# mozendr/FHE-SPEAR

Hardware: AMD Instinct MI355X
Metric: BSGS matvecs/sec at d=2048,N=16384,L0=36; sec/RWKV-block at 1/2/4/8 GPU (higher is better)
Workload: dtype u64

## Files before the change

fhe-spear_amd/csrc/fhs_host.hip:

```cpp
#include <execinfo.h>
#include <hip/hip_runtime.h>
#include <unistd.h>

#include <algorithm>
#include <csignal>
#include <atomic>
#include <cmath>
#include <complex>
#include <cstdio>
#include <cstring>
#include <map>
#include <unordered_map>
#include <chrono>
#include <memory>
#include <mutex>
#include <set>
#include <string>
#include <thread>
#include <vector>

#include "../../include/fhespear.h"
#include "fhs_kernels.h"
#include "fhs_modarith.h"
#include "fhs_tables.h"
// ... 47 lines not shown
    if (!bits || !out || n <= 0 || N < 2 || (N & (N - 1))) return fail(FHS_ERR_INVALID, "create_coeff_modulus: bad args");
    for (int i = 0; i < n; ++i)
        if (bits[i] < 2 || bits[i] > 61) return fail(FHS_ERR_INVALID, "create_coeff_modulus: bit size must be in [2, 61]");
    if (!coeff_modulus_search(N, bits, n, out)) return fail(FHS_ERR_INVALID, "create_coeff_modulus: not enough primes");
    return FHS_OK;
}
extern "C" uint64_t fhs_galois_elt_from_step(int step, uint64_t N) { return galois_elt_from_step(step, N); }

struct PendingRot {
    KsItem item;
    fhs_ciphertext* out;
    const fhs_ciphertext* in;
};

struct fhs_context {
    int device = 0;
    hipStream_t st = nullptr;
    fhs::KsSide side{};
    std::recursive_mutex mu;
    uint64_t N = 0;
    int logN = 0, L0 = 0, P = 0, K = 0, dnum = 0;
    std::vector<uint64_t> q;
    std::vector<uint64_t> elts;
    DevTables T{};
    std::vector<void*> tables;
    void* items_dev = nullptr;
    void* ptrs_dev = nullptr;
    std::vector<PendingRot> pending;
    int pending_l = -1;
    std::set<const void*> pending_refs;
    std::set<const void*> pending_outs;
    int debug_fail_flushes = 0;
    int debug_fail_alloc = -1;
    std::vector<std::complex<double>> fft_w;
    std::vector<std::complex<double>> dec_twist;
    std::vector<uint64_t> slot_index;
    std::atomic<uint64_t> bytes_live{0};
    std::atomic<int> refs{1};
    std::unordered_map<size_t, std::vector<void*>> free_blocks;
    std::unordered_map<const void*, uint64_t*> key_a;
    size_t cached_bytes = 0;
    size_t cache_cap = 0;
    uint64_t cache_tick = 0;
    std::unordered_map<size_t, uint64_t> size_tick;
    uint64_t evicted_blocks = 0, fit_hits = 0, seal_corr_drops = 0;
    uint32_t timer_mask = 0;
    std::vector<hipEvent_t> timer_open;
    std::vector<std::vector<std::pair<hipEvent_t, hipEvent_t>>> timer_pairs;
    fhs::KTimer ktimer{};
    unsigned char* ring = nullptr;
    size_t ring_head = 0;
    int ring_seg = 0;
    static constexpr size_t kRingBytes = 16u << 20;
    static constexpr int kRingSegs = 8;
    static constexpr size_t kSegBytes = kRingBytes / kRingSegs;
    hipEvent_t ring_ev[kRingSegs] = {};
    uint64_t ring_waits = 0, ring_blocked = 0;
    fhs::Stager stager{};
    std::map<std::pair<int, int>, std::vector<uint64_t>> crt_cache;
    double* readback = nullptr;
    size_t readback_bytes = 0;
    std::map<std::pair<const uint64_t*, int>, uint64_t*> seal_corr;
    size_t seal_corr_bytes = 0;
    size_t seal_corr_cap = 0;
    fhs::SealHoist seal_hoist{};
    enum { SCR_KS, SCR_BSGS_INNER, SCR_BSGS_WS, SCR_BSGS_SUM, SCR_RESCALE, SCR_ENC_PTRS, SCR_COUNT };
// ... 1185 lines not shown
    return export_dev(c, pd, pt_bytes(pt), host);
}
extern "C" fhs_status fhs_ciphertext_import(fhs_context* c, const uint64_t* host, int ncomp, int ci, double scale,
                                            fhs_ciphertext** out) {
    ENTER(c);
    if (!host || !out || ncomp < 2 || ncomp > 3) return fail(FHS_ERR_INVALID, "ciphertext_import: bad args");
    NEW_CT(ct, ncomp, ci, scale);
    HIPCHK(hipMemcpyAsync(ct->d, host, ct_bytes(ct.p), hipMemcpyHostToDevice, c->st), "ciphertext_import");
    HIPCHK(hipStreamSynchronize(c->st), "ciphertext_import");
    *out = ct.release();
    return FHS_OK;
}
extern "C" fhs_status fhs_plaintext_import(fhs_context* c, const uint64_t* host, int ci, double scale,
                                           fhs_plaintext** out) {
    ENTER(c);
    if (!host || !out) return fail(FHS_ERR_INVALID, "plaintext_import: bad args");
    NEW_PT(pt, ci, scale);
    HIPCHK(hipMemcpyAsync(pt->d, host, pt_bytes(pt.p), hipMemcpyHostToDevice, c->st), "plaintext_import");
    HIPCHK(hipStreamSynchronize(c->st), "plaintext_import");
    *out = pt.release();
    return FHS_OK;
}
extern "C" fhs_status fhs_debug_fail_next_flushes(fhs_context* c, int count) {
    if (!c || count < 0) return fail(FHS_ERR_INVALID, "debug_fail_next_flushes: bad args");
    Guard g(c);
    c->debug_fail_flushes = count;
    return FHS_OK;
}
extern "C" fhs_status fhs_debug_force_fork(fhs_context* c, int on, uint64_t* forked) {
    if (!c) return fail(FHS_ERR_INVALID, "debug_force_fork: null context");
    Guard g(c);
    if (on >= 0) c->side.min_wg = on ? 0 : fhs::kForkMinWg;
    if (forked) *forked = c->side.forked;
    return FHS_OK;
}
extern "C" fhs_status fhs_debug_fail_alloc(fhs_context* c, int nth, int* was_armed) {
    if (!c) return fail(FHS_ERR_INVALID, "debug_fail_alloc: null context");
    Guard g(c);
    if (was_armed) *was_armed = c->debug_fail_alloc >= 0;
    c->debug_fail_alloc = nth < 0 ? -1 : nth;
    return FHS_OK;
}
extern "C" fhs_status fhs_debug_alloc_stats(fhs_context* c, uint64_t* out, int n) {
    if (!c || !out || n < 0) return fail(FHS_ERR_INVALID, "debug_alloc_stats: bad args");
    Guard g(c);
    const uint64_t v[FHS_ALLOC_STATS_COUNT] = {c->cached_bytes,    c->cache_cap,     c->evicted_blocks, c->fit_hits,
                                               c->seal_corr_bytes, c->seal_corr_cap, c->seal_corr_drops};
    for (int i = 0; i < n && i < FHS_ALLOC_STATS_COUNT; ++i) out[i] = v[i];
    return FHS_OK;
}
extern "C" fhs_status fhs_debug_launch_ledger(int op, char* buf, uint64_t len, uint64_t* needed) {
    if (op == FHS_LEDGER_ARM || op == FHS_LEDGER_DISARM) {
        fhs::ledger_arm(op == FHS_LEDGER_ARM);
        return FHS_OK;
    }
    if (op != FHS_LEDGER_READ) return fail(FHS_ERR_INVALID, "debug_launch_ledger: unknown operation");
    const std::string names = fhs::ledger_read();
    if (needed) *needed = names.size() + 1;
    if (!buf || len < names.size() + 1) return fail(FHS_ERR_INVALID, "debug_launch_ledger: buffer too short");
    memcpy(buf, names.c_str(), names.size() + 1);
    return FHS_OK;
}
extern "C" fhs_status fhs_ciphertext_device_ptr(const fhs_ciphertext* ct, void** dptr, uint64_t* bytes) {
    if (!ct || !dptr) return fail(FHS_ERR_INVALID, "null argument");
    fhs_context* c = ct->ctx;
    Guard g(c);
// ... 1204 lines not shown
        if (!baby[b] || baby[b]->l != l || baby[b]->ncomp != 2 || baby[b]->ci != ci)
            return fail(FHS_ERR_LEVEL, "bsgs: baby steps and diagonals must share one chain index");
        LIVE(baby[b]);
    }
    if (rescale && l < 2) return fail(FHS_ERR_LEVEL, "bsgs: no level left for the final rescale");
    if (giant_elts && giant_elts[0] != 1) return fail(FHS_ERR_INVALID, "linear_transform: giant group 0 must be the identity");
    HostTrace ht;
    std::vector<const uint64_t*> keys(Beff, nullptr), akeys(Beff, nullptr);
    for (int g = 1; g < Beff; ++g) {
        const uint64_t elt = giant_elts ? giant_elts[g] : fhs_galois_elt_from_step(g * G, c->N);
        auto it = gk->keys.find(elt);
        if (it == gk->keys.end()) return fail(FHS_ERR_KEY, "bsgs: galois key for a giant step is missing");
        keys[g] = it->second;
        akeys[g] = key_akey(c, it->second);
    }
    const size_t S = (size_t)l * c->N;
    std::vector<const uint64_t*> ptrs(G + D);
    for (int b = 0; b < G; ++b) ptrs[b] = baby[b]->d;
    for (int k = 0; k < D; ++k) ptrs[G + k] = pt_ptrs[k];
    ht.mark("keys+ptrs");
    HIPCHK(stage_h2d(c, c->ptrs_dev, ptrs.data(), sizeof(void*) * (G + D)), "bsgs");
    ht.mark("stage ptrs");
    const uint64_t* const* dbaby = reinterpret_cast<const uint64_t* const*>(c->ptrs_dev);
    const uint64_t* const* dpts = dbaby + G;
    uint64_t* inner = nullptr;
    HIPCHK(scratch(c, fhs_context::SCR_BSGS_INNER, 8ull * Beff * 2 * S, &inner), "bsgs inner products");
    const fhs::KTimer* tm = ktimer(c);
    const size_t wsb = std::max<size_t>(8, fhs::bsgs_workspace_bytes(c->T, Beff - 1, l));
    uint64_t* ws = nullptr;
    HIPCHK(scratch(c, fhs_context::SCR_BSGS_WS, wsb, &ws), "bsgs workspace");
    uint64_t* sum = nullptr;
    HIPCHK(scratch(c, fhs_context::SCR_BSGS_SUM, 16 * S, &sum), "bsgs sum");
    ht.mark("workspaces");
    HIPCHK(fhs::launch_bsgs(c->T, dbaby, dpts, G, Beff, D, l, keys.data(), akeys.data(), giant_elts, inner, sum, ws, wsb,
                            c->items_dev, c->stager, c->st, tm, ptl, &c->side),
           "bsgs");
    ht.mark("launch bsgs");
    if (!rescale) {
        NEW_CT(r, 2, ci, baby[0]->scale * pt_scale);
        HIPCHK(hipMemcpyAsync(r->d, sum, 8 * 2 * S, hipMemcpyDeviceToDevice, c->st), "linear_transform");
        *out = r.release();
        return FHS_OK;
    }
    NEW_CT(r, 2, ci + 1, baby[0]->scale * pt_scale / (double)c->q[l - 1]);
    uint64_t* scr = nullptr;
    HIPCHK(scratch(c, fhs_context::SCR_RESCALE, 16ull * c->N, &scr), "bsgs rescale");
    HIPCHK(fhs::launch_rescale(c->T, sum, r->d, scr, 2, l, c->st, tm), "bsgs rescale");
    ht.mark("rescale+frees");
    *out = r.release();
    return FHS_OK;
}

static int pts_ptl(const fhs_context* c, const fhs_plaintext* const* pts, int D) {
    static const bool dense = getenv("FHESPEAR_BSGS_DENSE") != nullptr;
    if (dense || D < 1 || c->T.max_qbits > 59 || !pts[0]->dc) return 0;
    for (int k = 1; k < D; ++k)
        if (!pts[k]->dc || pts[k]->tlog != pts[0]->tlog) return 0;
    return pts[0]->tlog;
}
extern "C" fhs_status fhs_bsgs_multiply_accumulate(fhs_context* c, const fhs_ciphertext* const* baby, int G,
                                                   const fhs_plaintext* const* pts, int D, int B,
                                                   const fhs_galois_keys* gk, fhs_ciphertext** out) {
    ENTER(c);
    if (!pts || !gk || !out || !baby) return fail(FHS_ERR_INVALID, "null argument");
    std::vector<const uint64_t*> p(D);
    for (int k = 0; k < D; ++k) {
// ... 893 lines not shown
```

fhe-spear_amd/csrc/fhs_kernels.h:

```cpp
#pragma once
#include <hip/hip_runtime.h>
#include <stdint.h>

#include <string>

struct PrfKey;

namespace fhs {

typedef uint64_t u64;

struct DevTables {
    const void* primes;
    const u64* tw_fwd;
    const u64* tw_inv;
    const u64* modup_intt;
    const u64* modup_hat;
    const u64* modup_R;
    const u64* modup_Q;
    const u64* modup_xd;
    const u64* modup_xt;
    const u64* md_xd;
    const u64* md_intt;
    const u64* md_hat;
// ... 54 lines not shown

hipError_t launch_ntt_fwd(const DevTables& T, u64* data, int limbs, int l_split, int npoly, size_t poly_stride,
                          hipStream_t st);
hipError_t launch_ntt_inv(const DevTables& T, u64* data, int limbs, int l_split, int npoly, size_t poly_stride,
                          hipStream_t st);
hipError_t launch_eltwise(const DevTables& T, int op, const u64* a, const u64* b, u64* out, int ncomp, int l,
                          size_t a_cstride, size_t b_cstride, hipStream_t st);
hipError_t launch_tensor(const DevTables& T, const u64* const* a_dev, const u64* const* b_dev, const u64* a, const u64* b,
                         int R, u64* out3, int l, hipStream_t st);
hipError_t launch_rescale(const DevTables& T, const u64* in, u64* out, u64* scratch, int ncomp, int l,
                          hipStream_t st, const KTimer* tm = nullptr);
hipError_t launch_rescale_many(const DevTables& T, const u64* const* ins_dev, const u64* const* mul_dev, int count, int l,
                               u64* out, u64* scratch, hipStream_t st, const KTimer* tm = nullptr);
struct Stager {
    void* user;
    hipError_t (*h2d)(void* user, void* dst, const void* src, size_t bytes);
};
constexpr int kForkMinWg = 8 * 256;
struct KsSide {
    hipStream_t st = nullptr;
    hipEvent_t fork = nullptr, join = nullptr;
    int min_wg = kForkMinWg;
    unsigned long long forked = 0;
};
hipError_t launch_keyswitch(const DevTables& T, const KsItem* items_host, int R, const u64* const* uniq_host, int U,
                            int l, u64* workspace, size_t ws_bytes, void* items_dev, const Stager& sg, hipStream_t st,
                            const KTimer* tm, SealHoist* sh = nullptr);
size_t keyswitch_workspace_bytes(const DevTables& T, int R, int U, int l);

size_t bsgs_workspace_bytes(const DevTables& T, int R, int l);
hipError_t launch_bsgs(const DevTables& T, const u64* const* baby_dev, const u64* const* pts_dev, int G, int B, int D,
                       int l, const u64* const* keys_host, const u64* const* akeys_host, const u64* giant_elts, u64* inner,
                       u64* out, u64* workspace, size_t ws_bytes, void* items_dev, const Stager& sg, hipStream_t st,
                       const KTimer* tm, int ptl = 0, KsSide* side = nullptr);
hipError_t launch_bsgs_inner(const DevTables& T, const u64* const* baby_dev, const u64* const* pts_dev, int G, int g0,
                             int g1, int D, int l, u64* inner, hipStream_t st, int ptl = 0);
hipError_t launch_dot_tensor(const DevTables& T, const u64* const* q_dev, const u64* const* db_dev, int J, int C, int l,
                             u64* out3, hipStream_t st, const KTimer* tm = nullptr);
hipError_t launch_encode(const DevTables& T, const double* vals, int count, size_t n, size_t stride, bool is_real,
                         double scale, u64* const* outs_dev, int l, hipStream_t st,
                         double* coef_scratch = nullptr, const unsigned char* tlog = nullptr,
                         u64* const* couts_dev = nullptr, int ss = 0);
hipError_t launch_enc_period(const double* vals, int count, size_t n, size_t stride, bool is_real, int smax,
                             unsigned char* tlog, hipStream_t st);
int encode_sparse_max_log(int logN);
hipError_t launch_expand_compact(const u64* dc, u64* d, int l, int N, int tl, hipStream_t st);
hipError_t launch_sample(const DevTables& T, int mode, const ::PrfKey& K, u64 sid, u64* out, int l, hipStream_t st,
                         int npoly = 1, u64 sid_step = 0, u64* const* outs_dev = nullptr);
hipError_t launch_switch_key_assemble(const DevTables& T, u64* b_out, const u64* a, const u64* e_ntt, const u64* s_ntt,
                                      const u64* snew_ntt, int digit, hipStream_t st);
hipError_t launch_galois_perm(const DevTables& T, const u64* in, u64* out, int limbs, u64 elt, hipStream_t st);
hipError_t launch_encrypt_sym_batch(const DevTables& T, const ::PrfKey& K, u64 sid_mask, u64 sid_err, u64 sid_step,
                                    u64* const* cts_dev, const u64* s, const u64* const* pts_dev, int count, int l,
                                    signed char* small, u64* eb, hipStream_t st, const double* coef = nullptr);
hipError_t launch_encode_coef(const DevTables& T, const double* vals, int count, size_t n, size_t stride, bool is_real,
                              double scale, double* coef, hipStream_t st, const unsigned char* tlog = nullptr);
hipError_t launch_encrypt_pk_batch(const DevTables& T, const ::PrfKey& K, u64 sid, u64 sid_step, u64* cts,
                                   const u64* pk0, const u64* pk1, const u64* const* pts_dev, const u64* pt,
                                   const double* coef, int count, int l, signed char* small, u64* ub, hipStream_t st,
                                   const KTimer* tm = nullptr);
hipError_t launch_encrypt_combine(const DevTables& T, int mode, u64* c0, u64* c1, const u64* s_or_pk0, const u64* pk1,
                                  const u64* u_ntt, const u64* e0, const u64* e1, const u64* pt, int l, hipStream_t st);
hipError_t launch_decrypt(const DevTables& T, const u64* ct, int ncomp, const u64* s, u64* out, int l, hipStream_t st);
hipError_t launch_decrypt_many(const DevTables& T, const u64* const* cts_dev, int count, int ncomp, const u64* s, u64* out,
                               size_t out_stride, int l, hipStream_t st);
hipError_t launch_diag_gather(const double* M1, const double* M2, int D, int G, int n, int k0, int rows, int trans,
                              double* out, hipStream_t st);
// ... 54 lines not shown
```

fhe-spear_amd/csrc/fhs_kernels.hip:

```cpp
#include "fhs_kernels.h"
typedef unsigned long long u64x2_t __attribute__((ext_vector_type(2)));
#ifndef FHS_MODUP_STORE_AUX
#define FHS_MODUP_STORE_AUX 2
#endif
#ifndef FHS_KSIP_UNROLL
#define FHS_KSIP_UNROLL 4
#endif
#include "fhs_ntt.h"
#include "fhs_buffer.h"
#include "fhs_xcdmap.h"

#include <atomic>
#include <cxxabi.h>
#include <mutex>
#include <set>
#include <string>
#include <cstdio>
#include <cstdlib>
#include <cstring>
#include <vector>
#include <algorithm>

#define FHS_INNER_WAVES 16
#define FHS_INNER_VEC 2
// ... 471 lines not shown
    const int vecs = wg2 >= 8 * 256 ? 2 : 1;
    FHS_LAUNCH(k_tensor, dim3((T.N + 512 * vecs - 1) / (512 * vecs), l, R), dim3(256), 0, st, T, a_dev, b_dev, a, b, out3, l,
               vecs);
    return hipGetLastError();
}

__global__ void k_key_prod(DevTables T, const u64* a, const u64* b, u64* out, int limbs) {
    const size_t S = (size_t)limbs * T.N;
    for (size_t idx = blockIdx.x * (size_t)blockDim.x + threadIdx.x; idx < S; idx += (size_t)gridDim.x * blockDim.x) {
        const PrimeK& P = PK(T, (int)(idx / T.N));
        out[idx] = mulmod(a[idx], b[idx], P);
    }
}
hipError_t launch_key_prod(const DevTables& T, const u64* a, const u64* b, u64* out, int limbs, hipStream_t st) {
    FHS_LAUNCH(k_key_prod, dim3(eltwise_grid((size_t)limbs * T.N)), dim3(256), 0, st, T, a, b, out, limbs);
    return hipGetLastError();
}

__global__ void k_galois_perm(DevTables T, const u64* in, u64* out, int limbs, u64 elt) {
    const size_t S = (size_t)limbs * T.N;
    for (size_t idx = blockIdx.x * (size_t)blockDim.x + threadIdx.x; idx < S; idx += (size_t)gridDim.x * blockDim.x) {
        const size_t base = idx - idx % T.N;
        out[idx] = in[base + galois_src((int)(idx % T.N), elt, T.logN)];
    }
}
hipError_t launch_galois_perm(const DevTables& T, const u64* in, u64* out, int limbs, u64 elt, hipStream_t st) {
    FHS_LAUNCH(k_galois_perm, dim3(eltwise_grid((size_t)limbs * T.N)), dim3(256), 0, st, T, in, out, limbs,
               elt);
    return hipGetLastError();
}

template <int LOGN, bool H = ntt_half<LOGN>()>
__global__ void __launch_bounds__((ntt_threads<LOGN, H>())) k_rescale_intt(DevTables T, const u64* in, const u64* const* ins,
                                                                      const u64* const* mul, u64* scratch, int l) {
    constexpr int N = 1 << LOGN;
    __shared__ __attribute__((aligned(16))) u64 lds[ntt_lds_words<LOGN, H>()];
    const int comp = blockIdx.x, pi = l - 1;
    const PrimeK& P = PK(T, pi);
    const u64* src = ins ? ins[comp >> 1] + ((size_t)(comp & 1) * l + pi) * N : in + ((size_t)comp * l + pi) * N;
    u64* dst = scratch + (size_t)comp * N;
    const u64 half = P.q >> 1, q = P.q;
    const u64* tw = T.tw_inv + (size_t)pi * N * 2;
    auto store = [&](int e, u64 v) { dst[e] = addmod(v, half, q); };
    if (mul) {
        const u64* pt = mul[comp >> 1] + (size_t)pi * N;
        inv_limb<LOGN, FHS_NTT_RL, H>(lds, threadIdx.x, tw, q, P.ninv, P.ninv_s, P.w1ninv, P.w1ninv_s,
                                   [&](int e) { return mulmod(src[e], pt[e], P); }, store);
    } else {
        inv_limb<LOGN, FHS_NTT_RL, H>(lds, threadIdx.x, tw, q, P.ninv, P.ninv_s, P.w1ninv, P.w1ninv_s,
                                   [&](int e) { return src[e]; }, store);
    }
}
template <int LOGN, bool H = ntt_half<LOGN>()>
__global__ void __launch_bounds__((ntt_threads<LOGN, H>())) k_rescale_ntt(DevTables T, const u64* in, const u64* const* ins,
                                                                     const u64* const* mul, const u64* scratch, u64* out,
                                                                     int l) {
    constexpr int N = 1 << LOGN;
    __shared__ __attribute__((aligned(16))) u64 lds[ntt_lds_words<LOGN, H>()];
    const int i = blockIdx.x, comp = blockIdx.y;
    const PrimeK& P = PK(T, i);
    const RedU RU = redu(P);
    const u64* rs = T.rescale + ((size_t)l * T.L0 + i) * 4;
    const u64 inv = rs[0], inv_s = rs[1], hq = rs[2], q = RU.q;
    const u64* src = scratch + (size_t)comp * N;
    const u64* a = ins ? ins[comp >> 1] + ((size_t)(comp & 1) * l + i) * N : in + ((size_t)comp * l + i) * N;
    u64* o = out + ((size_t)comp * (l - 1) + i) * N;
    const u64* tw = T.tw_fwd + (size_t)i * N * 2;
    auto load = [&](int e) { return submod(reduce64(src[e], P), hq, q); };
    if (mul) {
        const u64* pt = mul[comp >> 1] + (size_t)i * N;
        fwd_limb<LOGN, FHS_NTT_RL, H>(lds, threadIdx.x, tw, RU, load, [&](int e, u64 t) {
            o[e] = shoup(submod(mulmod(a[e], pt[e], P), t, q), inv, inv_s, q);
        });
    } else {
        fwd_limb<LOGN, FHS_NTT_RL, H>(lds, threadIdx.x, tw, RU, load,
                                   [&](int e, u64 t) { o[e] = shoup(submod(a[e], t, q), inv, inv_s, q); });
    }
// ... 60 lines not shown
    if constexpr (WLX) {
        const int wb = wl_base<LOGN - 1, 16, 8>(tid), wp = lds_pad(wb);
#pragma unroll
        for (int c = 0; c < 16; ++c) {
            const int off = wl_off<LOGN - 1, 16, 8>(c);
            const int e = g * NH + wb + off;
            o[e] = shoup(submod(a[e], fwd_canon(lds[wp + off + off / 16], RU), q), inv, inv_s, q);
        }
    } else {
#pragma unroll
        for (int c = 0; c < 16; ++c) {
            const int e = g * NH + tid + c * TH;
            o[e] = shoup(submod(a[e], fwd_canon(lds[row_pad<TH>(tid, c)], RU), q), inv, inv_s, q);
        }
    }
}
#ifndef FHS_SPLIT_MAX_WG
#define FHS_SPLIT_MAX_WG 256
#endif
hipError_t launch_rescale(const DevTables& T, const u64* in, u64* out, u64* scratch, int ncomp, int l,
                          hipStream_t st, const KTimer* tm) {
    FHS_TMARK(tm, KID_RESCALE, 1, st);
    FHS_DISPATCH_LOGN(T.logN, {
        if constexpr (LOGN == 15) {
            if (ncomp <= 2) {
                FHS_LAUNCH((k_rescale_intt_hs<LOGN>), dim3(2, ncomp), dim3(ntt_threads<LOGN, true>()), 0, st, T,
                           in, scratch, l);
                FHS_LAUNCH((k_rescale_ntt_hs<LOGN>), dim3(l - 1, ncomp, 2), dim3(ntt_threads<LOGN, true>()), 0, st,
                           T, in, scratch, out, l);
                break;
            }
        }
        constexpr const u64* const* none = nullptr;
        FHS_NTT_LAUNCH(k_rescale_intt, ncomp, dim3(ncomp), st, T, in, none, none, scratch, l);
        FHS_NTT_LAUNCH(k_rescale_ntt, (l - 1) * ncomp, dim3(l - 1, ncomp), st, T, in, none, none, scratch, out, l);
    });
    FHS_TMARK(tm, KID_RESCALE, 0, st);
    return hipGetLastError();
}

hipError_t launch_rescale_many(const DevTables& T, const u64* const* ins_dev, const u64* const* mul_dev, int count, int l,
                               u64* out, u64* scratch, hipStream_t st, const KTimer* tm) {
    if (!ins_dev || count < 1 || 2 * (size_t)count > 65535 || l < 2 || l > 65536) return hipErrorInvalidValue;
    const int ncomp = 2 * count;
    FHS_TMARK(tm, KID_RESCALE, 1, st);
    FHS_DISPATCH_LOGN(T.logN, {
        constexpr const u64* none = nullptr;
        FHS_NTT_LAUNCH(k_rescale_intt, ncomp, dim3(ncomp), st, T, none, ins_dev, mul_dev, scratch, l);
        FHS_NTT_LAUNCH(k_rescale_ntt, (l - 1) * ncomp, dim3(l - 1, ncomp), st, T, none, ins_dev, mul_dev, scratch, out, l);
    });
    FHS_TMARK(tm, KID_RESCALE, 0, st);
    return hipGetLastError();
}

hipError_t launch_last_limbs_intt(const DevTables& T, const u64* const* ins_dev, int count, int l, u64* dco, hipStream_t st,
                                  const KTimer* tm) {
    if (count < 1 || count > 65535 || l < 1) return hipErrorInvalidValue;
    FHS_TMARK(tm, KID_WSUM_INTT, 1, st);
    FHS_DISPATCH_LOGN(T.logN, {
        FHS_NTT_LAUNCH(k_rescale_intt, 2 * count, dim3(2 * count), st, T, static_cast<const u64*>(nullptr), ins_dev,
                       static_cast<const u64* const*>(nullptr), dco, l);
    });
    FHS_TMARK(tm, KID_WSUM_INTT, 0, st);
    return hipGetLastError();
}

template <int LOGN>
__global__ void __launch_bounds__((1 << LOGN) / 16) k_ks_intt(DevTables T, const u64* const* uniq, u64* acoef, int l, int U) {
    constexpr int N = 1 << LOGN, TH = N / 16;
    __shared__ __attribute__((aligned(16))) u64 lds[ntt_lds_words<LOGN, false>()];
    const int tid = threadIdx.x;
    int i, u;
    if (!plain_tm(blockIdx.x, l, U, i, u)) return;
    const PrimeK& P = PK(T, i);
    const u64* src = uniq[u] + (size_t)i * N;
#pragma unroll
    for (int c = 0; c < 16; ++c) lds[row_pad<TH>(tid, c)] = src[tid + c * TH];
    __syncthreads();
    const u64* cst = T.modup_intt + ((size_t)l * T.L0 + i) * 4;
    ntt_inv_lds<LOGN, FHS_NTT_RL>(lds, tid, T.tw_inv + (size_t)i * N * 2, P.q, cst[0], cst[1], cst[2], cst[3]);
    u64* dst = acoef + ((size_t)u * l + i) * N;
#pragma unroll
    for (int k = 0; k < 16; ++k) dst[tid + k * TH] = csub(lds[row_pad<TH>(tid, k)], P.q);
}

template <int LOGN>
__global__ void __launch_bounds__((1 << LOGN) / 32, 4) k_ks_intt_h(DevTables T, const u64* const* uniq, u64* acoef,
                                                                   int l, int U) {
    constexpr int N = 1 << LOGN, NH = N / 2, TH = N / 32;
    __shared__ __attribute__((aligned(16))) u64 lds[(1 << (LOGN - 1)) + (1 << (LOGN - 1)) / 16];
    const int tid = threadIdx.x;
    int i, u;
    if (!plain_tm(blockIdx.x, l, U, i, u)) return;
    const PrimeK& P = PK(T, i);
// ... 1253 lines not shown
        }
#pragma unroll
        for (int j = 0; j < FHS_GSUM_RB; ++j) {
#pragma unroll
            for (int k = 0; k < PMAX; ++k) {
                if (k < P_) {
                    ylo[k] += v[j][k];
                    yhi[k] += ylo[k] < v[j][k];
                }
            }
        }
    }
    for (int i = i0; i < i1; ++i) {
        const PrimeK& P = PK(T, i);
        const u64 q = P.q;
        u128 cs = {0, 0};
#pragma unroll
        for (int k = 0; k < PMAX; ++k)
            if (k < P_) mac128(cs, reduce128(ylo[k], yhi[k], P), T.md_hat[(size_t)k * T.L0 + i]);
        if (T.ks_seal) {
            u128 h = {0, 0};
            mac128(h, (u64)R, T.md_pinv[3 * T.L0 + i]);
            const u64 rh = reduce128(h.lo, h.hi, P);
            cs.lo = reduce128(cs.lo, cs.hi, P);
            cs.hi = 0;
            cs.lo = submod(cs.lo, rh, q);
        }
        u64 cv = reduce128(cs.lo, cs.hi, P);
        convsum[(size_t)comp * S + (size_t)i * N + n] = cv;
    }
}
template <int LOGN, bool H = ntt_half<LOGN>()>
__global__ void __launch_bounds__((ntt_threads<LOGN, H>())) k_giant_final(DevTables T, const u64* bpart, const u64* inner0,
                                                                     const u64* convsum, u64* out, int l) {
    constexpr int N = 1 << LOGN;
    __shared__ __attribute__((aligned(16))) u64 lds[ntt_lds_words<LOGN, H>()];
    const int i = blockIdx.x, comp = blockIdx.y;
    const PrimeK& P = PK(T, i);
    const RedU RU = redu(P);
    const size_t off = ((size_t)comp * l + i) * N, boff = ((size_t)comp * (l + T.P) + i) * N;
    const u64 pinv = T.md_pinv[2 * i], pinv_s = T.md_pinv[2 * i + 1], q = RU.q;
    fwd_limb<LOGN, FHS_NTT_RL, H>(lds, threadIdx.x, T.tw_fwd + (size_t)i * N * 2, RU,
                               [&](int e) { return convsum[off + e]; },
                               [&](int e, u64 v) {
                                   out[off + e] = submod(addmod(bpart[boff + e], inner0[off + e], q),
                                                         shoup(v, pinv, pinv_s, q), q);
                               });
}

size_t bsgs_workspace_bytes(const DevTables& T, int R, int l) {
    return keyswitch_workspace_bytes(T, R, R, l) + 8 * (size_t)T.N * 4 * l;
}

template <class Each>
static hipError_t lds_opt_in(std::atomic<bool>& done, size_t bytes, Each each) {
    if (done.load(std::memory_order_acquire)) return hipSuccess;
    hipError_t e = hipSuccess;
    each([&](const void* k) {
        if (k && e == hipSuccess) e = hipFuncSetAttribute(k, hipFuncAttributeMaxDynamicSharedMemorySize, (int)bytes);
    });
    if (e == hipSuccess) done.store(true, std::memory_order_release);
    return e;
}

constexpr int kInnerWindow = 64;
typedef void (*InnerFn)(DevTables, const u64* const*, const u64* const*, int, int, int, int, int, int, u64*);
template <int VEC, int WAVES, int FOLD, int TL>
static InnerFn inner_kernel_acc(bool acc) {
    return acc ? k_bsgs_inner<VEC, WAVES, FOLD, true, TL> : k_bsgs_inner<VEC, WAVES, FOLD, false, TL>;
}
template <int VEC, int WAVES>
static InnerFn inner_kernel(bool fold16, bool acc, int ptl) {
    if (!fold16) return ptl == 0 ? inner_kernel_acc<VEC, WAVES, 8, 0>(acc) : nullptr;
    switch (ptl) {
        case 0: return inner_kernel_acc<VEC, WAVES, 16, 0>(acc);
        case 1: return inner_kernel_acc<VEC, WAVES, 16, 1>(acc);
        case 2: return inner_kernel_acc<VEC, WAVES, 16, 2>(acc);
        case 3: return inner_kernel_acc<VEC, WAVES, 16, 3>(acc);
    }
    return nullptr;
}
template <int VEC, int WAVES>
static hipError_t launch_inner_t(const DevTables& T, const u64* const* baby, const u64* const* pts, int G, int g0,
                                 int g1, int D, int l, u64* inner, hipStream_t st, int ptl) {
    constexpr int W = 64 * VEC;
    static std::atomic<bool> opted{false};
    hipError_t e = lds_opt_in(opted, (size_t)kInnerWindow * 2 * W * 8, [](auto f) {
        for (int fold16 = 0; fold16 < 2; ++fold16)
            for (int acc = 0; acc < 2; ++acc)
                for (int tl = 0; tl <= 3; ++tl)
                    f(reinterpret_cast<const void*>(inner_kernel<VEC, WAVES>(fold16, acc, tl)));
    });
    if (e != hipSuccess) return e;
    if (ptl < 0 || ptl > 3 || (ptl > 0 && (T.max_qbits > 59 || VEC != 2))) return hipErrorInvalidValue;
    for (int b0 = 0; b0 < G; b0 += kInnerWindow) {
        const int Gw = std::min(kInnerWindow, G - b0), Dw = D - b0;
// ... 101 lines not shown
template <int VEC, int WAVES>
static hipError_t launch_dot_t(const DevTables& T, const u64* const* q, const u64* const* db, int J, int C, int l, u64* out,
                               hipStream_t st) {
    constexpr int W = 64 * VEC;
    static std::atomic<bool> opted{false};
    hipError_t e = lds_opt_in(opted, (size_t)kDotWindowMax * 2 * W * 8, [](auto f) {
        for (int fold16 = 0; fold16 < 2; ++fold16)
            for (int acc = 0; acc < 2; ++acc) f(reinterpret_cast<const void*>(dot_kernel<VEC, WAVES>(fold16, acc)));
    });
    if (e != hipSuccess) return e;
    for (int j0 = 0; j0 < J; j0 += kDotWindowMax) {
        const int Jw = std::min(kDotWindowMax, J - j0);
        const size_t lds = (size_t)Jw * 2 * W * 8;
        const dim3 grid(T.N / W, l), block(64 * WAVES);
        const DotFn k = dot_kernel<VEC, WAVES>(T.max_qbits <= 59, j0 > 0);
        FHS_LAUNCH(k, grid, block, lds, st, T, q + j0, db + j0, J, Jw, C, l, out);
        e = hipGetLastError();
        if (e != hipSuccess) return e;
    }
    return hipSuccess;
}
hipError_t launch_dot_tensor(const DevTables& T, const u64* const* q_dev, const u64* const* db_dev, int J, int C, int l,
                             u64* out3, hipStream_t st, const KTimer* tm) {
    if (T.N % (64 * FHS_DOT_VEC) || J < 1 || C < 1) return hipErrorInvalidValue;
    FHS_TMARK(tm, KID_DOT_TENSOR, 1, st);
    const hipError_t e = launch_dot_t<FHS_DOT_VEC, FHS_DOT_WAVES>(T, q_dev, db_dev, J, C, l, out3, st);
    FHS_TMARK(tm, KID_DOT_TENSOR, 0, st);
    return e;
}

hipError_t launch_bsgs(const DevTables& T, const u64* const* baby_dev, const u64* const* pts_dev, int G, int B, int D,
                       int l, const u64* const* keys_host, const u64* const* akeys_host, const u64* giant_elts, u64* inner,
                       u64* out, u64* ws, size_t ws_bytes, void* items_dev, const Stager& sg, hipStream_t st,
                       const KTimer* tm, int ptl, KsSide* side) {
    const int R = B - 1;
    const size_t N = T.N, S = (size_t)l * N;
    if (T.N % 128 || G < 1 || R > 512) return hipErrorInvalidValue;
    if (R > 0 && bsgs_workspace_bytes(T, R, l) > ws_bytes) return hipErrorInvalidValue;
    KsItem items[512];
    const u64* uniq[512];
    for (int r = 0; r < R; ++r) {
        const int g = r + 1;
        const u64* ct = inner + (size_t)g * 2 * S;
        u64 elt = 1;
        if (giant_elts) elt = giant_elts[g];
        else
            for (int s2 = 0; s2 < g * G; ++s2) elt = (elt * 5) & (2 * N - 1);
        items[r] = KsItem{ct + S, ct, nullptr, keys_host[g], nullptr, nullptr, elt, (u64)r,
                          akeys_host ? akeys_host[g] : nullptr};
        uniq[r] = ct + S;
    }
    std::vector<KsItem> seal_orig;
    u64* seal_perm = ws + ks_core_bytes(T, R, R, l) / 8;
    if (T.ks_seal && R > 0) {
        seal_orig.assign(items, items + R);
        seal_rewrite(T, items, R, uniq, l, seal_perm);
    }
    const KsItem* it = nullptr;
    const u64* const* uq = nullptr;
    if (R > 0) {
        hipError_t e = upload_items(items, R, uniq, R, items_dev, sg, &it, &uq);
        if (e != hipSuccess) return e;
    }
    hipError_t he = hipSuccess;
    if (pts_dev) {
        FHS_TMARK(tm, KID_BSGS_INNER, 1, st);
        he = launch_inner_t<FHS_INNER_VEC, FHS_INNER_WAVES>(T, baby_dev, pts_dev, G, 0, B, D, l, inner, st, ptl);
        FHS_TMARK(tm, KID_BSGS_INNER, 0, st);
        if (he != hipSuccess) return he;
    }
// ... 7 lines not shown
    FHS_DISPATCH_LOGN(T.logN, {
        const KsBufs b = ks_carve(T, ws, R, R, l);
        const int E = l + T.P, dn = (E - 1) / T.P;
        SideFork sf(side, st);
        auto special_chain = [&](hipStream_t cs) {
            ks_ip_stage(T, it, uq, R, l, b, cs, tm, l, E);
            ks_special_intt_stage<LOGN>(T, R, l, b, cs, tm);
            FHS_TMARK(tm, KID_GIANT_SUM, 1, cs);
            FHS_LAUNCH(k_giant_sum, dim3((T.N + 255) / 256, 2, (l + FHS_GSUM_ICH - 1) / FHS_GSUM_ICH), dim3(256), 0, cs, T,
                       b.ycoef, convsum, l, R);
            FHS_TMARK(tm, KID_GIANT_SUM, 0, cs);
        };
        ks_intt_stage<LOGN>(T, uq, R, l, b, st, tm);
        if (!side_forks(side, LOGN, (long long)l * dn * R)) {
            ks_modup_stage<LOGN>(T, uq, R, l, b, st, tm);
            special_chain(st);
            giant_ip_sum_stage(T, it, uq, R, l, b, st, tm);
        } else {
            if constexpr (ks_uses_half(LOGN)) {
                FHS_TMARK(tm, KID_MODUP, 1, st);
                launch_modup<LOGN>(T, uq, b.acoef, b.vcnt, b.ext, l, R, st, kModupSpecial);
                FHS_TMARK(tm, KID_MODUP, 0, st);
                ge = sf.fork();
                if (ge == hipSuccess) {
                    special_chain(side->st);
                    FHS_TMARK(tm, KID_MODUP, 1, st);
                    launch_modup<LOGN>(T, uq, b.acoef, b.vcnt, b.ext, l, R, st, kModupData);
                    FHS_TMARK(tm, KID_MODUP, 0, st);
                    giant_ip_sum_stage(T, it, uq, R, l, b, st, tm);
                    ge = sf.join();
                }
            }
        }
        if (ge == hipSuccess) {
            FHS_TMARK(tm, KID_GIANT_FINAL, 1, st);
            FHS_NTT_LAUNCH(k_giant_final, l * 2, dim3(l, 2), st, T, b.acc, inner, convsum, out, l);
            FHS_TMARK(tm, KID_GIANT_FINAL, 0, st);
        }
    });
    if (ge != hipSuccess) return ge;
    return hipGetLastError();
}



__device__ __forceinline__ u64 rnd_testdata(u64 key, u64 ctr) { return sm64(key ^ sm64(ctr ^ 0xD1B54A32D192ED03ULL)); }

__global__ void k_sample(DevTables T, int mode, PrfKey K, u64 sid, u64* out, int l, u64 sid_step, u64* const* outs) {
    const int N = T.N;
    const size_t S = (size_t)l * N;
    sid += blockIdx.y * sid_step;
    out = outs ? outs[blockIdx.y] : out + blockIdx.y * S;
    for (size_t idx = blockIdx.x * (size_t)blockDim.x + threadIdx.x; idx < S; idx += (size_t)gridDim.x * blockDim.x) {
        const int i = (int)(idx / N), n = (int)(idx % N);
        const PrimeK& P = PK(T, i);
        u64 v;
        if (mode == SAMPLE_UNIFORM) {
            u64 hi, lo;
            prf128(K, sid, (uint32_t)idx, hi, lo);
            v = reduce128(lo, hi, P);
        } else if (mode == SAMPLE_SEEDED) {
            v = seeded_uniform_x(sid + seeded_ctr_mix(i, n), P.q, 64 - __clzll(P.q));
        } else if (mode == SAMPLE_TESTDATA) {
            const u64 ctr = 2 * ((u64)i * N + n);
            v = reduce128(rnd_testdata(sid, ctr + 1), rnd_testdata(sid, ctr), P);
        } else {
            u64 r, unused;
            prf128(K, sid, (uint32_t)n, r, unused);
            long long s;
// ... 1021 lines not shown
```

fhe-spear_amd/python/pyPhantom/__init__.py:

```python
from __future__ import annotations

import ctypes as C
import enum
import os
import sys
import threading
from pathlib import Path

import numpy as np

__version__ = "fhespear-mi355x-0.1"

_HERE = Path(__file__).resolve().parent
_LIB_CANDIDATES = [
    os.environ.get("FHESPEAR_LIB", ""),
    str(_HERE.parent.parent / "lib" / "libfhespear_hip.so"),
]


def _share_torch_hip_runtime():
    if os.environ.get("FHESPEAR_HIP_RUNTIME", "torch") != "torch":
        return None
    import importlib.util
    try:
# ... 121 lines not shown
    "fhs_bsgs_giant_steps_device": (C.c_int, [_vp, _vp, C.c_int, C.c_int, C.c_double, _u64p, _vp, C.POINTER(_vp)]),
    "fhs_linear_transform": (C.c_int, [_vp, C.POINTER(_vp), C.c_int, C.POINTER(_vp), C.c_int, C.c_int, _u64p, _vp,
                                       C.c_int, C.POINTER(_vp)]),
    "fhs_weighted_sums": (C.c_int, [_vp, C.POINTER(_vp), C.c_int, _dblp, C.c_int64, C.c_int, C.c_double, C.POINTER(_vp)]),
    "fhs_debug_wsum_round": (C.c_int, [_u64, _u64p, _u64p, C.c_int, C.POINTER(C.c_int64), _u64p]),
    "fhs_debug_wsum_accumulate": (C.c_int, [_u64, _u64p, _u64p, C.c_int, _u64, _u64, _u64p]),
    "fhs_multiply_const": (C.c_int, [_vp, _vp, C.c_double, C.c_double, C.POINTER(_vp)]),
    "fhs_add_const": (C.c_int, [_vp, _vp, C.c_double, C.POINTER(_vp)]),
    "fhs_mod_raise": (C.c_int, [_vp, _vp, C.POINTER(_vp)]),
    "fhs_bootstrap_evalmod": (C.c_int, [_vp, _vp, _vp, _dblp, _dblp, C.c_int, C.c_int, C.c_int, C.POINTER(_vp)]),
    "fhs_encode_precise": (C.c_int, [_vp, _dblp, C.c_size_t, C.c_size_t, C.c_double, C.c_int, C.POINTER(_vp)]),
    "fhs_encode_diagonals": (C.c_int, [_vp, _dblp, _dblp, C.c_int, C.c_int, C.c_double, C.c_int, C.POINTER(_vp)]),
    "fhs_encode_diagonals_ex": (C.c_int, [_vp, _vp, _vp, C.c_int64, C.c_int, C.c_int, C.c_int, C.c_double, C.c_int,
                                          C.POINTER(_vp)]),
    "fhs_encode_diagonals_rows": (C.c_int, [_vp, _vp, _vp, C.c_int64, C.c_int, C.c_int, C.c_int, C.c_double, C.c_int,
                                            _vp, C.c_int, C.POINTER(_vp)]),
    "fhs_host_alloc": (C.c_int, [_u64, C.POINTER(_vp)]),
    "fhs_host_free": (C.c_int, [_vp]),
    "fhs_random_plaintexts": (C.c_int, [_vp, _u64, C.c_int, C.c_int, C.c_double, C.POINTER(_vp)]),
    "fhs_event_record": (C.c_int, [_vp, C.POINTER(_vp)]),
    "fhs_event_elapsed": (C.c_int, [_vp, _vp, C.POINTER(C.c_float)]),
    "fhs_event_destroy": (C.c_int, [_vp]),
    "fhs_kernel_timer": (C.c_int, [_vp, C.c_int, C.POINTER(C.c_float), _ip, C.c_int]),
    "fhs_kernel_timer_arm": (C.c_int, [_vp, C.c_uint32]),
    "fhs_ciphertext_copy_to_device": (C.c_int, [_vp, _vp, _vp]),
    "fhs_ciphertext_from_device": (C.c_int, [_vp, _vp, C.c_int, C.c_int, C.c_double, C.POINTER(_vp)]),
    "fhs_ciphertext_copy_to_device_async": (C.c_int, [_vp, _vp, _vp]),
    "fhs_ciphertext_from_device_async": (C.c_int, [_vp, _vp, C.c_int, C.c_int, C.c_double, C.POINTER(_vp)]),
    "fhs_context_stream": (C.c_int, [_vp, C.POINTER(_vp)]),
    "fhs_staging_stats": (C.c_int, [_vp, C.POINTER(C.c_uint64), C.POINTER(C.c_uint64)]),
    "fhs_debug_fail_next_flushes": (C.c_int, [_vp, C.c_int]),
    "fhs_debug_fail_alloc": (C.c_int, [_vp, C.c_int, _ip]),
    "fhs_debug_force_fork": (C.c_int, [_vp, C.c_int, _u64p]),
    "fhs_debug_launch_ledger": (C.c_int, [C.c_int, C.c_char_p, _u64, _u64p]),
    "fhs_debug_alloc_stats": (C.c_int, [_vp, _u64p, C.c_int]),
}
_OPTIONAL = {
    "fhs_bsgs_multiply_accumulate": ("bsgs_multiply_accumulate",),
    "fhs_bsgs_from_cpu": ("bsgs_from_cpu", "bsgs_complete_from_cpu"),
    "fhs_upload_plaintexts": ("upload_plaintexts",),
    "fhs_offload_plaintexts": ("offload_plaintexts",),
    "fhs_encode_real_batch": ("ckks_encoder.encode_double_vector_batch",),
    "fhs_encode_batch": ("ckks_encoder.encode_complex_vector_batch",),
}
_DISABLED = {x.strip() for x in os.environ.get("FHESPEAR_DISABLE_SYMBOLS", "").split(",") if x.strip()}
_MISSING = []
for _name, (_res, _args) in _SIGS.items():
    try:
        if _name in _DISABLED:
            raise AttributeError(_name)
        _f = getattr(_lib, _name)
    except AttributeError:
        if _name in _OPTIONAL:
            _MISSING.append(_name)
            continue
        raise ImportError(f"pyPhantom: {LIB_PATH} lacks the required symbol {_name}") from None
    _f.restype = _res
    _f.argtypes = _args

_OOM, _HIP, _NODEV = 2, 3, 7


def _check(rc: int, what: str = ""):
    if rc == 0:
        return
    msg = (_lib.fhs_last_error() or b"").decode(errors="replace")
# ... 956 lines not shown

def kernel_timer_read(ctx, reset=False):
    out = {}
    for name, kid in KERNEL_IDS.items():
        ms, n = C.c_float(), C.c_int()
        _check(_lib.fhs_kernel_timer(ctx._h, kid, C.byref(ms), C.byref(n), 0), "kernel_timer")
        out[name] = (float(ms.value), int(n.value))
    if reset:
        _check(_lib.fhs_kernel_timer(ctx._h, -1, None, None, 1), "kernel_timer")
    return out


def stage_timer_read(ctx, reset=False):
    out = {}
    for name, kid in STAGE_IDS.items():
        ms, n = C.c_float(), C.c_int()
        _check(_lib.fhs_kernel_timer(ctx._h, kid, C.byref(ms), C.byref(n), 0), "kernel_timer")
        out[name] = (float(ms.value), int(n.value))
    if reset:
        _check(_lib.fhs_kernel_timer(ctx._h, -1, None, None, 1), "kernel_timer")
    return out


def debug_fail_next_flushes(ctx, count=1):
    _check(_lib.fhs_debug_fail_next_flushes(ctx._h, int(count)), "debug_fail_next_flushes")


def debug_force_fork(ctx, on=None):
    n = C.c_uint64(0)
    _check(_lib.fhs_debug_force_fork(ctx._h, -1 if on is None else int(bool(on)), C.byref(n)), "debug_force_fork")
    return int(n.value)


def debug_fail_alloc(ctx, nth):
    was = C.c_int()
    _check(_lib.fhs_debug_fail_alloc(ctx._h, int(nth), C.byref(was)), "debug_fail_alloc")
    return bool(was.value)


def debug_launch_ledger(op="read"):
    ops = {"arm": 0, "disarm": 1, "read": 2}
    if op not in ops:
        raise ValueError(f"debug_launch_ledger: op must be one of {sorted(ops)}")
    if op != "read":
        _check(_lib.fhs_debug_launch_ledger(ops[op], None, 0, None), "debug_launch_ledger")
        return None
    need = _u64()
    _lib.fhs_debug_launch_ledger(2, None, 0, C.byref(need))
    while True:
        buf = C.create_string_buffer(int(need.value))
        if _lib.fhs_debug_launch_ledger(2, buf, len(buf), C.byref(need)) == 0:
            return buf.value.decode().splitlines()
        if int(need.value) <= len(buf):
            _check(1, "debug_launch_ledger")


def staging_stats(ctx):
    a, b = C.c_uint64(), C.c_uint64()
    _check(_lib.fhs_staging_stats(ctx._h, C.byref(a), C.byref(b)), "staging_stats")
    return int(a.value), int(b.value)


def ciphertext_copy_to_device(ctx, ct, dst_ptr, sync=True):
    fn = _lib.fhs_ciphertext_copy_to_device if sync else _lib.fhs_ciphertext_copy_to_device_async
    _check(fn(ctx._h, ct._h, _vp(int(dst_ptr))), "copy_to_device")

# ... 44 lines not shown
```

include/fhespear.h:

```cpp
#ifndef FHESPEAR_H
#define FHESPEAR_H
#include <stddef.h>
#include <stdint.h>

#ifdef __cplusplus
extern "C" {
#endif

typedef int fhs_status;
enum {
    FHS_OK = 0,
    FHS_ERR_INVALID = 1,
    FHS_ERR_OOM = 2,
    FHS_ERR_HIP = 3,
    FHS_ERR_LEVEL = 4,
    FHS_ERR_SCALE = 5,
    FHS_ERR_KEY = 6,
    FHS_ERR_NODEVICE = 7
};

typedef struct fhs_context fhs_context;
typedef struct fhs_ciphertext fhs_ciphertext;
typedef struct fhs_plaintext fhs_plaintext;
typedef struct fhs_secret_key fhs_secret_key;
typedef struct fhs_public_key fhs_public_key;
typedef struct fhs_relin_key fhs_relin_key;
typedef struct fhs_galois_keys fhs_galois_keys;

const char* fhs_last_error(void);
const char* fhs_version(void);
int fhs_device_count(void);
fhs_status fhs_device_pci_bus_id(int device, char* buf, int len);
fhs_status fhs_debug_fail_next_flushes(fhs_context* ctx, int count);
fhs_status fhs_debug_fail_alloc(fhs_context* ctx, int nth, int* was_armed);
fhs_status fhs_debug_force_fork(fhs_context* ctx, int on, uint64_t* forked);
enum { FHS_LEDGER_ARM = 0, FHS_LEDGER_DISARM = 1, FHS_LEDGER_READ = 2 };
fhs_status fhs_debug_launch_ledger(int op, char* buf, uint64_t len, uint64_t* needed);
enum {
    FHS_ALLOC_CACHED_BYTES = 0,
    FHS_ALLOC_CACHE_CAP = 1,
    FHS_ALLOC_EVICTED = 2,
    FHS_ALLOC_FIT = 3,
    FHS_ALLOC_SEAL_CORR_BYTES = 4,
    FHS_ALLOC_SEAL_CORR_CAP = 5,
    FHS_ALLOC_SEAL_CORR_DROPS = 6,
    FHS_ALLOC_STATS_COUNT = 7
};
fhs_status fhs_debug_alloc_stats(fhs_context* ctx, uint64_t* out, int n);

fhs_status fhs_create_coeff_modulus(uint64_t N, const int* bit_sizes, int n, uint64_t* primes_out);
uint64_t fhs_galois_elt_from_step(int step, uint64_t N);

fhs_status fhs_context_create(uint64_t N, const uint64_t* primes, int nprimes, int special,
                              const uint64_t* galois_elts, int n_elts, int device, fhs_context** out);
fhs_status fhs_context_destroy(fhs_context* ctx);
fhs_status fhs_context_info(const fhs_context* ctx, uint64_t* N, int* L0, int* P, int* n_elts);
fhs_status fhs_context_galois_elts(const fhs_context* ctx, uint64_t* elts_out);
fhs_status fhs_synchronize(fhs_context* ctx);
fhs_status fhs_memory_in_use(fhs_context* ctx, uint64_t* bytes);

fhs_status fhs_secret_key_create(fhs_context* ctx, const uint8_t* key32 ,
                                 fhs_secret_key** out);
fhs_status fhs_secret_key_destroy(fhs_secret_key* sk);
fhs_status fhs_gen_public_key(fhs_context* ctx, fhs_secret_key* sk, fhs_public_key** out);
fhs_status fhs_gen_relin_key(fhs_context* ctx, fhs_secret_key* sk, fhs_relin_key** out);
fhs_status fhs_create_galois_keys(fhs_context* ctx, fhs_secret_key* sk, const uint64_t* elts, int n,
                                  fhs_galois_keys** out);
fhs_status fhs_public_key_destroy(fhs_public_key* pk);
// ... 161 lines not shown
```

Before: 162.9.

## Fuse BSGS giant-step final accumulation with the rescale

```diff
diff --git a/fhe-spear_amd/csrc/fhs_host.hip b/fhe-spear_amd/csrc/fhs_host.hip
--- a/fhe-spear_amd/csrc/fhs_host.hip
+++ b/fhe-spear_amd/csrc/fhs_host.hip
@@ -103,6 +103,8 @@
     std::set<const void*> pending_outs;
     int debug_fail_flushes = 0;
     int debug_fail_alloc = -1;
+    int chain_fusion = 1;
+    uint64_t chain_fused = 0;
     std::vector<std::complex<double>> fft_w;
     std::vector<std::complex<double>> dec_twist;
     std::vector<uint64_t> slot_index;
@@ -1354,6 +1356,13 @@
     Guard g(c);
     if (on >= 0) c->side.min_wg = on ? 0 : fhs::kForkMinWg;
     if (forked) *forked = c->side.forked;
+    return FHS_OK;
+}
+extern "C" fhs_status fhs_debug_chain_fusion(fhs_context* c, int mode, uint64_t* taken) {
+    if (!c || mode < -1 || mode > 2) return fail(FHS_ERR_INVALID, "debug_chain_fusion: bad args");
+    Guard g(c);
+    if (mode >= 0) c->chain_fusion = mode;
+    if (taken) *taken = c->chain_fused;
     return FHS_OK;
 }
 extern "C" fhs_status fhs_debug_fail_alloc(fhs_context* c, int nth, int* was_armed) {
@@ -2624,6 +2633,18 @@
     uint64_t* sum = nullptr;
     HIPCHK(scratch(c, fhs_context::SCR_BSGS_SUM, 16 * S, &sum), "bsgs sum");
     ht.mark("workspaces");
+    if (rescale && c->chain_fusion > 0 && fhs::bsgs_rescale_fuses(c->T, Beff, l)) {
+        NEW_CT(r, 2, ci + 1, baby[0]->scale * pt_scale / (double)c->q[l - 1]);
+        uint64_t* scr = nullptr;
+        HIPCHK(scratch(c, fhs_context::SCR_RESCALE, 16ull * c->N, &scr), "bsgs rescale");
+        HIPCHK(fhs::launch_bsgs(c->T, dbaby, dpts, G, Beff, D, l, keys.data(), akeys.data(), giant_elts, inner, sum, ws,
+                                wsb, c->items_dev, c->stager, c->st, tm, ptl, &c->side, r->d, scr),
+               "bsgs");
+        ++c->chain_fused;
+        ht.mark("launch bsgs");
+        *out = r.release();
+        return FHS_OK;
+    }
     HIPCHK(fhs::launch_bsgs(c->T, dbaby, dpts, G, Beff, D, l, keys.data(), akeys.data(), giant_elts, inner, sum, ws, wsb,
                             c->items_dev, c->stager, c->st, tm, ptl, &c->side),
            "bsgs");
diff --git a/fhe-spear_amd/csrc/fhs_kernels.h b/fhe-spear_amd/csrc/fhs_kernels.h
--- a/fhe-spear_amd/csrc/fhs_kernels.h
+++ b/fhe-spear_amd/csrc/fhs_kernels.h
@@ -110,7 +110,8 @@
 hipError_t launch_bsgs(const DevTables& T, const u64* const* baby_dev, const u64* const* pts_dev, int G, int B, int D,
                        int l, const u64* const* keys_host, const u64* const* akeys_host, const u64* giant_elts, u64* inner,
                        u64* out, u64* workspace, size_t ws_bytes, void* items_dev, const Stager& sg, hipStream_t st,
-                       const KTimer* tm, int ptl = 0, KsSide* side = nullptr);
+                       const KTimer* tm, int ptl = 0, KsSide* side = nullptr, u64* rescaled = nullptr, u64* vco = nullptr);
+bool bsgs_rescale_fuses(const DevTables& T, int B, int l);
 hipError_t launch_bsgs_inner(const DevTables& T, const u64* const* baby_dev, const u64* const* pts_dev, int G, int g0,
                              int g1, int D, int l, u64* inner, hipStream_t st, int ptl = 0);
 hipError_t launch_dot_tensor(const DevTables& T, const u64* const* q_dev, const u64* const* db_dev, int J, int C, int l,
diff --git a/fhe-spear_amd/csrc/fhs_kernels.hip b/fhe-spear_amd/csrc/fhs_kernels.hip
--- a/fhe-spear_amd/csrc/fhs_kernels.hip
+++ b/fhe-spear_amd/csrc/fhs_kernels.hip
@@ -527,7 +527,8 @@
 
 template <int LOGN, bool H = ntt_half<LOGN>()>
 __global__ void __launch_bounds__((ntt_threads<LOGN, H>())) k_rescale_intt(DevTables T, const u64* in, const u64* const* ins,
-                                                                      const u64* const* mul, u64* scratch, int l) {
+                                                                      const u64* const* mul, u64* scratch, int l,
+                                                                      const u64* inner0, const u64* convsum) {
     constexpr int N = 1 << LOGN;
     __shared__ __attribute__((aligned(16))) u64 lds[ntt_lds_words<LOGN, H>()];
     const int comp = blockIdx.x, pi = l - 1;
@@ -537,7 +538,15 @@
     const u64 half = P.q >> 1, q = P.q;
     const u64* tw = T.tw_inv + (size_t)pi * N * 2;
     auto store = [&](int e, u64 v) { dst[e] = addmod(v, half, q); };
-    if (mul) {
+    if (convsum) {
+        const size_t off = ((size_t)comp * l + pi) * N, boff = ((size_t)comp * (l + T.P) + pi) * N;
+        const u64 pinv = T.md_pinv[2 * pi], pinv_s = T.md_pinv[2 * pi + 1];
+        inv_limb<LOGN, FHS_NTT_RL, H>(lds, threadIdx.x, tw, q, P.ninv, P.ninv_s, P.w1ninv, P.w1ninv_s,
+                                   [&](int e) { return addmod(in[boff + e], inner0[off + e], q); },
+                                   [&](int e, u64 v) {
+                                       dst[e] = addmod(submod(v, shoup(convsum[off + e], pinv, pinv_s, q), q), half, q);
+                                   });
+    } else if (mul) {
         const u64* pt = mul[comp >> 1] + (size_t)pi * N;
         inv_limb<LOGN, FHS_NTT_RL, H>(lds, threadIdx.x, tw, q, P.ninv, P.ninv_s, P.w1ninv, P.w1ninv_s,
                                    [&](int e) { return mulmod(src[e], pt[e], P); }, store);
@@ -664,7 +673,8 @@
             }
         }
         constexpr const u64* const* none = nullptr;
-        FHS_NTT_LAUNCH(k_rescale_intt, ncomp, dim3(ncomp), st, T, in, none, none, scratch, l);
+        constexpr const u64* in0 = nullptr;
+        FHS_NTT_LAUNCH(k_rescale_intt, ncomp, dim3(ncomp), st, T, in, none, none, scratch, l, in0, in0);
         FHS_NTT_LAUNCH(k_rescale_ntt, (l - 1) * ncomp, dim3(l - 1, ncomp), st, T, in, none, none, scratch, out, l);
     });
     FHS_TMARK(tm, KID_RESCALE, 0, st);
@@ -678,7 +688,7 @@
     FHS_TMARK(tm, KID_RESCALE, 1, st);
     FHS_DISPATCH_LOGN(T.logN, {
         constexpr const u64* none = nullptr;
-        FHS_NTT_LAUNCH(k_rescale_intt, ncomp, dim3(ncomp), st, T, none, ins_dev, mul_dev, scratch, l);
+        FHS_NTT_LAUNCH(k_rescale_intt, ncomp, dim3(ncomp), st, T, none, ins_dev, mul_dev, scratch, l, none, none);
         FHS_NTT_LAUNCH(k_rescale_ntt, (l - 1) * ncomp, dim3(l - 1, ncomp), st, T, none, ins_dev, mul_dev, scratch, out, l);
     });
     FHS_TMARK(tm, KID_RESCALE, 0, st);
@@ -691,7 +701,8 @@
     FHS_TMARK(tm, KID_WSUM_INTT, 1, st);
     FHS_DISPATCH_LOGN(T.logN, {
         FHS_NTT_LAUNCH(k_rescale_intt, 2 * count, dim3(2 * count), st, T, static_cast<const u64*>(nullptr), ins_dev,
-                       static_cast<const u64* const*>(nullptr), dco, l);
+                       static_cast<const u64* const*>(nullptr), dco, l, static_cast<const u64*>(nullptr),
+                       static_cast<const u64*>(nullptr));
     });
     FHS_TMARK(tm, KID_WSUM_INTT, 0, st);
     return hipGetLastError();
@@ -2011,7 +2022,8 @@
 }
 template <int LOGN, bool H = ntt_half<LOGN>()>
 __global__ void __launch_bounds__((ntt_threads<LOGN, H>())) k_giant_final(DevTables T, const u64* bpart, const u64* inner0,
-                                                                     const u64* convsum, u64* out, int l) {
+                                                                     const u64* convsum, u64* out, int l,
+                                                                     const u64* vco) {
     constexpr int N = 1 << LOGN;
     __shared__ __attribute__((aligned(16))) u64 lds[ntt_lds_words<LOGN, H>()];
     const int i = blockIdx.x, comp = blockIdx.y;
@@ -2019,6 +2031,21 @@
     const RedU RU = redu(P);
     const size_t off = ((size_t)comp * l + i) * N, boff = ((size_t)comp * (l + T.P) + i) * N;
     const u64 pinv = T.md_pinv[2 * i], pinv_s = T.md_pinv[2 * i + 1], q = RU.q;
+    if (vco) {
+        const u64* rs = T.rescale + ((size_t)l * T.L0 + i) * 4;
+        const u64 inv = rs[0], inv_s = rs[1], hq = rs[2];
+        const u64* v = vco + (size_t)comp * N;
+        u64* o = out + ((size_t)comp * (l - 1) + i) * N;
+        fwd_limb<LOGN, FHS_NTT_RL, H>(lds, threadIdx.x, T.tw_fwd + (size_t)i * N * 2, RU,
+                                   [&](int e) {
+                                       return addmod(shoup(convsum[off + e], pinv, pinv_s, q),
+                                                     submod(reduce64(v[e], P), hq, q), q);
+                                   },
+                                   [&](int e, u64 t) {
+                                       o[e] = shoup(submod(addmod(bpart[boff + e], inner0[off + e], q), t, q), inv, inv_s, q);
+                                   });
+        return;
+    }
     fwd_limb<LOGN, FHS_NTT_RL, H>(lds, threadIdx.x, T.tw_fwd + (size_t)i * N * 2, RU,
                                [&](int e) { return convsum[off + e]; },
                                [&](int e, u64 v) {
@@ -2041,6 +2068,8 @@
     if (e == hipSuccess) done.store(true, std::memory_order_release);
     return e;
 }
+
+bool bsgs_rescale_fuses(const DevTables& T, int B, int l) { return B > 1 && l >= 2 && T.logN <= 14; }
 
 constexpr int kInnerWindow = 64;
 typedef void (*InnerFn)(DevTables, const u64* const*, const u64* const*, int, int, int, int, int, int, u64*);
@@ -2208,10 +2237,11 @@
 hipError_t launch_bsgs(const DevTables& T, const u64* const* baby_dev, const u64* const* pts_dev, int G, int B, int D,
                        int l, const u64* const* keys_host, const u64* const* akeys_host, const u64* giant_elts, u64* inner,
                        u64* out, u64* ws, size_t ws_bytes, void* items_dev, const Stager& sg, hipStream_t st,
-                       const KTimer* tm, int ptl, KsSide* side) {
+                       const KTimer* tm, int ptl, KsSide* side, u64* rescaled, u64* vco) {
     const int R = B - 1;
     const size_t N = T.N, S = (size_t)l * N;
     if (T.N % 128 || G < 1 || R > 512) return hipErrorInvalidValue;
+    if (rescaled && (!bsgs_rescale_fuses(T, B, l) || !vco)) return hipErrorInvalidValue;
     if (R > 0 && bsgs_workspace_bytes(T, R, l) > ws_bytes) return hipErrorInvalidValue;
     KsItem items[512];
     const u64* uniq[512];
@@ -2285,9 +2315,18 @@
                 }
             }
         }
-        if (ge == hipSuccess) {
+        constexpr const u64* none = nullptr;
+        if (ge == hipSuccess && !rescaled) {
             FHS_TMARK(tm, KID_GIANT_FINAL, 1, st);
-            FHS_NTT_LAUNCH(k_giant_final, l * 2, dim3(l, 2), st, T, b.acc, inner, convsum, out, l);
+            FHS_NTT_LAUNCH(k_giant_final, l * 2, dim3(l, 2), st, T, b.acc, inner, convsum, out, l, none);
+            FHS_TMARK(tm, KID_GIANT_FINAL, 0, st);
+        } else if (ge == hipSuccess) {
+            constexpr const u64* const* nolist = nullptr;
+            FHS_TMARK(tm, KID_RESCALE, 1, st);
+            FHS_NTT_LAUNCH(k_rescale_intt, 2, dim3(2), st, T, b.acc, nolist, nolist, vco, l, inner, convsum);
+            FHS_TMARK(tm, KID_RESCALE, 0, st);
+            FHS_TMARK(tm, KID_GIANT_FINAL, 1, st);
+            FHS_NTT_LAUNCH(k_giant_final, l * 2, dim3(l - 1, 2), st, T, b.acc, inner, convsum, rescaled, l, vco);
             FHS_TMARK(tm, KID_GIANT_FINAL, 0, st);
         }
     });
diff --git a/fhe-spear_amd/python/pyPhantom/__init__.py b/fhe-spear_amd/python/pyPhantom/__init__.py
--- a/fhe-spear_amd/python/pyPhantom/__init__.py
+++ b/fhe-spear_amd/python/pyPhantom/__init__.py
@@ -177,6 +177,7 @@
     "fhs_debug_fail_next_flushes": (C.c_int, [_vp, C.c_int]),
     "fhs_debug_fail_alloc": (C.c_int, [_vp, C.c_int, _ip]),
     "fhs_debug_force_fork": (C.c_int, [_vp, C.c_int, _u64p]),
+    "fhs_debug_chain_fusion": (C.c_int, [_vp, C.c_int, _u64p]),
     "fhs_debug_launch_ledger": (C.c_int, [C.c_int, C.c_char_p, _u64, _u64p]),
     "fhs_debug_alloc_stats": (C.c_int, [_vp, _u64p, C.c_int]),
 }
@@ -1199,6 +1200,12 @@
     return int(n.value)
 
 
+def debug_chain_fusion(ctx, mode=None):
+    n = C.c_uint64(0)
+    _check(_lib.fhs_debug_chain_fusion(ctx._h, -1 if mode is None else int(mode), C.byref(n)), "debug_chain_fusion")
+    return int(n.value)
+
+
 def debug_fail_alloc(ctx, nth):
     was = C.c_int()
     _check(_lib.fhs_debug_fail_alloc(ctx._h, int(nth), C.byref(was)), "debug_fail_alloc")
diff --git a/include/fhespear.h b/include/fhespear.h
--- a/include/fhespear.h
+++ b/include/fhespear.h
@@ -34,6 +34,7 @@
 fhs_status fhs_debug_fail_next_flushes(fhs_context* ctx, int count);
 fhs_status fhs_debug_fail_alloc(fhs_context* ctx, int nth, int* was_armed);
 fhs_status fhs_debug_force_fork(fhs_context* ctx, int on, uint64_t* forked);
+fhs_status fhs_debug_chain_fusion(fhs_context* ctx, int mode, uint64_t* taken);
 enum { FHS_LEDGER_ARM = 0, FHS_LEDGER_DISARM = 1, FHS_LEDGER_READ = 2 };
 fhs_status fhs_debug_launch_ledger(int op, char* buf, uint64_t len, uint64_t* needed);
 enum {
```

Result: slower. 158.1 (-2.9%).
